# kshedden/muscato

Measured on AMD Instinct MI355X. Metric: reads/sec (100 bp, multi-map) at 1/2/4/8 MI355X; confirm-kernel HBM GB/s vs peak, higher is better.
Workload: dtype u32

## Files before the change

### muscato_amd/api.py

```python
from __future__ import annotations

import ctypes
import json
from dataclasses import dataclass, field, asdict
from typing import List, Optional, Sequence, Tuple

import numpy as np

from . import _lib


class MuscatoError(RuntimeError):
    pass


@dataclass
class Config:
    ReadFileName: str = ""
    GeneFileName: str = ""
    GeneIdFileName: str = ""
    ResultsFileName: str = ""
    Windows: List[int] = field(default_factory=list)
    WindowWidth: int = 0
    BloomSize: int = 0
# ... 210 lines not shown
        self._check(self._lib.musc_reads_sort_unique(self._h, seqs_ptr, off_ptr, nreads, 1 if on_device else 0,
                                                     ctypes.byref(po), ctypes.byref(pu), ctypes.byref(nu)),
                    "musc_reads_sort_unique")
        try:
            order = np.ctypeslib.as_array(ctypes.cast(po, ctypes.POINTER(ctypes.c_uint32)), shape=(max(nreads, 1),))[:nreads].copy()
            ustart = np.ctypeslib.as_array(ctypes.cast(pu, ctypes.POINTER(ctypes.c_uint32)), shape=(nu.value + 1,)).copy()
        finally:
            self._lib.musc_free_u32(po)
            self._lib.musc_free_u32(pu)
        self.n_reads = int(nu.value)
        return order, ustart

    def load_reads_packed(self, seqs: Sequence[bytes]) -> None:
        buf, off = concat(seqs)
        packed, mask = pack_2bit(buf, int(off[-1]))
        packed = np.concatenate([packed, np.zeros(8, np.uint8)])
        mp = mask.ctypes.data if mask is not None else None
        self._check(self._lib.musc_reads_load_packed(self._h, packed.ctypes.data, mp, off.ctypes.data, len(off) - 1),
                    "musc_reads_load_packed")
        self.n_reads = len(off) - 1

    def load_reads_packed_ptr(self, bases_ptr: int, mask_ptr: int, off_ptr: int, nreads: int) -> None:
        self._check(self._lib.musc_reads_load_packed(self._h, bases_ptr, mask_ptr or None, off_ptr, nreads),
                    "musc_reads_load_packed")
        self.n_reads = nreads

    def load_reads_packed32_ptr(self, bases_ptr: int, mask_ptr: int, lengths_ptr: int, fixed_len: int, nreads: int,
                                async_upload: bool = False) -> None:
        self._check(self._lib.musc_reads_load_packed32(self._h, bases_ptr, mask_ptr or None, lengths_ptr or None,
                                                       fixed_len, nreads, 1 if async_upload else 0),
                    "musc_reads_load_packed32")
        self.n_reads = nreads

    def match_device(self, cfg: Config, apply_mmtol: bool = True, skip_block_check: bool = False,
                     n_shards: int = 1) -> int:
        p = cfg.to_params(apply_mmtol, skip_block_check, n_shards)
        self._apply_partition_bases(cfg)
        n = ctypes.c_uint64()
        self._check(self._lib.musc_match_device(self._h, ctypes.byref(p), ctypes.byref(n)), "musc_match_device")
        return int(n.value)

    def hits_to(self, ptr: int, capacity: int, on_device: bool) -> None:
        self._check(self._lib.musc_hits_copy(self._h, ptr, capacity, 1 if on_device else 0), "musc_hits_copy")

    def hits_to_packed(self, ptr: int, capacity: int, on_device: bool, bits: Sequence[int], read_base: int = 0) -> None:
        b = (ctypes.c_int32 * 4)(*bits)
        self._check(self._lib.musc_hits_copy_packed(self._h, ptr, capacity, 1 if on_device else 0, read_base, b),
                    "musc_hits_copy_packed")

    def hits_to_compact(self, words_ptr: int, words_cap: int, counts_ptr: int, counts_cap: int, on_device: bool,
                        bits: Sequence[int]) -> None:
        b = (ctypes.c_int32 * 3)(*bits)
        self._check(self._lib.musc_hits_copy_compact(self._h, words_ptr, words_cap, counts_ptr, counts_cap,
                                                     1 if on_device else 0, b), "musc_hits_copy_compact")

    def unpack_hits(self, src_ptr: int, n: int, on_device: bool, bits: Sequence[int], dst_ptr: int) -> None:
        b = (ctypes.c_int32 * 4)(*bits)
        self._check(self._lib.musc_hits_unpack(self._h, src_ptr, n, 1 if on_device else 0, b, dst_ptr), "musc_hits_unpack")

    def match(self, cfg: Config, apply_mmtol: bool = True, n_shards: int = 1) -> np.ndarray:
        n = self.match_device(cfg, apply_mmtol, n_shards=n_shards)
        out = np.zeros((n, 4), dtype=np.uint32)
        if n:
            self.hits_to(out.ctypes.data, n, False)
        return out

    def overflow_probes(self) -> np.ndarray:
        pr, pw, n = ctypes.c_void_p(), ctypes.c_void_p(), ctypes.c_uint64()
        self._check(self._lib.musc_overflow_probes(self._h, ctypes.byref(pr), ctypes.byref(pw), ctypes.byref(n)),
                    "musc_overflow_probes")
        out = np.zeros((n.value, 2), dtype=np.uint32)
        if n.value:
            out[:, 0] = np.ctypeslib.as_array(ctypes.cast(pr, ctypes.POINTER(ctypes.c_uint32)), shape=(n.value,))
            out[:, 1] = np.ctypeslib.as_array(ctypes.cast(pw, ctypes.POINTER(ctypes.c_uint32)), shape=(n.value,))
        self._lib.musc_free_u32(pr)
        self._lib.musc_free_u32(pw)
        return out

    def last_instance(self) -> dict:
        w = (ctypes.c_uint32 * 4)()
        self._check(self._lib.musc_last_instance(self._h, w), "musc_last_instance")
        return {"path": "fused" if w[0] else "two-kernel" if w[1] else "none",
                "match": decode_instance(w[0]), "screen": decode_instance(w[1]), "confirm": decode_instance(w[2]),
                "block_mode": w[3] & 0xFF, "exact_rerun": bool(w[3] & 0x100)}

    def stats(self) -> dict:
        s = _lib.MuscStats()
        self._check(self._lib.musc_get_stats(self._h, ctypes.byref(s)), "musc_get_stats")
        return {k: getattr(s, k) for k, _ in s._fields_}


_INST_FIELDS = {1: ("k_match_t", ("W", "XM", "WIDE", "SG")), 2: ("k_match_g", (None, None, None, "SG")),
                3: ("k_screen", ("mask", "one", "lines")), 4: ("k_screen_t", ()), 5: ("k_confirm", ("mask", "w2"))}


def decode_instance(word: int) -> Optional[dict]:
    if not word:
        return None
    name, fields = _INST_FIELDS[word & 0xFF]
    d = {"kernel": name, "RW": (word >> 8) & 0xFF}
    for i, f in enumerate(fields):
        if f:
            d[f] = (word >> (16 + 4 * i)) & 0xF
    return d


def instance_name(d: Optional[dict]) -> str:
    return "none" if d is None else "%s<%s>" % (d["kernel"], ", ".join(str(v) for k, v in d.items() if k != "kernel"))


def instances() -> List[dict]:
    lib = _lib.load()
    n = ctypes.c_uint32()
    if lib.musc_instances(None, 0, ctypes.byref(n)):
        raise RuntimeError("musc_instances failed")
    buf = (ctypes.c_uint32 * max(1, n.value))()
    lib.musc_instances(buf, n.value, ctypes.byref(n))
    return [decode_instance(w) for w in buf[:n.value]]


def stream_plan(nreads: int, fixed_len: int, batch_reads: int = 16 << 20) -> dict:
    lib = _lib.load()
    n, planned = ctypes.c_uint64(), ctypes.c_uint64()
    if lib.musc_stream_plan(nreads, fixed_len, batch_reads, None, None, 0, ctypes.byref(n), ctypes.byref(planned)):
        raise ValueError("musc_stream_plan: %d reads of %d bases is not a read set the loader takes" % (nreads, fixed_len))
    ends = np.zeros(max(1, n.value), dtype=np.uint64)
    flags = np.zeros(max(1, n.value), dtype=np.uint8)
    lib.musc_stream_plan(nreads, fixed_len, batch_reads, ends.ctypes.data, flags.ctypes.data, n.value, ctypes.byref(n),
                         ctypes.byref(planned))
    ends, flags = ends[:n.value], flags[:n.value]
    return {"piece_ends": ends, "batch_ends": ends[flags != 0], "planned_batches": int(planned.value)}


def gather(engines: Sequence["Engine"], read_bases: Sequence[int], rccl: bool = False) -> np.ndarray:
    lib = engines[0]._lib
    n = len(engines)
    arr = (ctypes.c_void_p * n)(*[e._h for e in engines])
    bases = (ctypes.c_uint64 * n)(*[int(b) for b in read_bases])
    ph, cnt = ctypes.c_void_p(), ctypes.c_uint64()
    rc = lib.musc_gather_rccl(arr, n, bases, ctypes.byref(ph), ctypes.byref(cnt)) if rccl else 1
    if rccl and rc == 2:
        raise MuscatoError("musc_gather_rccl failed (%d): %s" % (rc, lib.musc_last_error(engines[0]._h).decode()))
    if rc != 0:
        rc = lib.musc_gather(arr, n, bases, ctypes.byref(ph), ctypes.byref(cnt))
    if rc != 0:
        raise MuscatoError("musc_gather failed (%d): %s" % (rc, lib.musc_last_error(engines[0]._h).decode()))
    out = np.zeros((cnt.value, 4), dtype=np.uint32)
    if cnt.value:
        ctypes.memmove(out.ctypes.data, ph, cnt.value * 16)
    lib.musc_free_hits(ph)
    return out


def sorted_hits(a: np.ndarray) -> np.ndarray:
    if len(a) == 0:
        return a.reshape(0, 4)
    idx = np.lexsort((a[:, 3], a[:, 2], a[:, 1], a[:, 0]))
    return a[idx]
```

### muscato_amd/csrc/kernels_match_lane.hpp

```cpp
#pragma once
#include "kernels_match_lane_inst.hpp"
#if defined(MUSC_LANE_DBG) && !defined(MUSC_LANE_DBG_SLOTS)
#define MUSC_LANE_DBG_SLOTS 3
#endif

template <int RW, int NW>
DEV void read_image_n(const Rec<RW>& rec, uint32_t sh, uint32_t (&img)[NW]) {
  const uint32_t bs = sh & 31u;
#define MUSC_IMG_W(Q) (((Q) >= 0 && (Q) < RW - 1) ? rec.w[((Q) >= 0 && (Q) < RW - 1) ? (Q) : 0] : 0u)
#define MUSC_IMG_CASE(WO)                                                  \
  case WO:                                                                 \
    _Pragma("unroll") for (int j = 0; j < NW; j++) {                       \
      const uint32_t hi = MUSC_IMG_W(j - WO), lo = MUSC_IMG_W(j - WO - 1); \
      img[j] = bs ? ((hi << bs) | (lo >> (32u - bs))) : hi;                \
    }                                                                      \
    break;
  switch (__builtin_amdgcn_readfirstlane((int)(sh >> 5))) {
    MUSC_IMG_CASE(0) MUSC_IMG_CASE(1) MUSC_IMG_CASE(2) MUSC_IMG_CASE(3)
    MUSC_IMG_CASE(4) MUSC_IMG_CASE(5) MUSC_IMG_CASE(6) MUSC_IMG_CASE(7)
    MUSC_IMG_CASE(8) MUSC_IMG_CASE(9) MUSC_IMG_CASE(10) MUSC_IMG_CASE(11) MUSC_IMG_CASE(12)
    default:
#pragma unroll
      for (int j = 0; j < NW; j++) img[j] = 0u;
      break;
  }
#undef MUSC_IMG_CASE
#undef MUSC_IMG_W
}


DEV void put_tuple(uint4* __restrict__ dst, uint32_t a, uint32_t b, uint32_t c, uint32_t d) { *dst = make_uint4(a, b, c, d); }

template <int RW, int W, int XM, bool WIDE, int SG>
__global__ __launch_bounds__(TILE, MATCHT_WAVES) void k_match_t(const uint32_t* __restrict__ rd, uint64_t r0, uint32_t n,
                                                                const MatchParams* __restrict__ mp,
                                                                const uint16_t* __restrict__ nmiss_tab,
                                                                const CtxBucket* __restrict__ T, const CtxEntry* __restrict__ E,
                                                                uint4* __restrict__ stage, uint64_t stage_cap,
                                                                uint4* __restrict__ spill, uint64_t spill_cap,
                                                                uint32_t* __restrict__ tbase, uint32_t* __restrict__ tcount2,
                                                                int block_mode, uint32_t block_thr,
                                                                uint32_t* __restrict__ block_table,
                                                                unsigned long long* __restrict__ counters,
                                                                const uint32_t* __restrict__ rdx) {
  static_assert(W >= 1 && W <= CTX_MAX_W, "context buckets serve at most CTX_MAX_W windows");
  constexpr bool RX = XM != 0, DBX = XM == 2;
  constexpr int NWAVE = TILE / 64;
  constexpr int NIN = WIDE ? CTXW_INLINE : CTX_INLINE;
  constexpr uint32_t WLIST = RW >= 12 && MATCHT_WLIST > 64 ? 64u : (uint32_t)MATCHT_WLIST;
  typedef XPos<WIDE> XP;
  constexpr int NW = WIDE ? CTXW_WORDS : 8;
  constexpr int NQ = WIDE ? 3 : 2;
  constexpr int NT = WIDE ? 3 : 2;
  extern __shared__ uint32_t s_dyn[];
  __shared__ uint4 s_line[NWAVE][64 * 8];
  __shared__ __attribute__((aligned(16))) uint32_t s_rec[2][NWAVE][WT * RW];
  __shared__ uint32_t s_meta[2][NWAVE][WT];
  __shared__ uint32_t s_xp[RX ? 2 : 1][RX ? NWAVE : 1][RX ? WT : 1];
  __shared__ uint32_t s_best[2][NWAVE][WT];
  __shared__ uint3 s_list[2][NWAVE][WLIST];
  __shared__ uint32_t s_cb[NWAVE][2 * WT];
  __shared__ uint32_t s_oix[NWAVE][WT];
  __shared__ uint8_t s_own[NWAVE][WT];
  __shared__ uint16_t s_nm[CONF_NM];
  constexpr bool BB_LDS = (W == 3 && XM == 0 && RW <= 8);
  __shared__ uint32_t s_bbp[BB_LDS ? NWAVE : 1][BB_LDS ? W : 1][BB_LDS ? WT : 1];

  typedef SpecGeom<SG> SGm;
  constexpr bool SPEC = SGm::on;
  static_assert(!SPEC || (SGm::nwin == W && !WIDE && XM == 0 && SGm::ww <= 15), "a specialised instance is built for its geometry's window count, 120-base buckets, no X, a direct table of one-word keys");
  constexpr int S_WW = SGm::ww, S_CL = SGm::CL, S_L = SGm::L, S_MIND = SGm::min_dinuc;
  constexpr int S_WIN[CTX_MAX_W] = {SGm::win[0], SGm::win[1], SGm::win[2], SGm::win[3]};
  if constexpr (SPEC) {
    bool same = mp->ww == S_WW && mp->CL == S_CL && mp->min_dinuc == S_MIND && mp->direct == 1 && mp->bits == 2 * S_WW && mp->W == W;
#pragma unroll
    for (int k = 0; k < W; k++) same = same && mp->win[k] == S_WIN[k] && mp->need[k] == (1u << k) - 1u;
    if (!same) {
      if (threadIdx.x == 0) atomicOr(&counters[3], 8ull);
      return;
    }
  }
  const int ww = SPEC ? S_WW : mp->ww, CL = SPEC ? S_CL : mp->CL, min_dinuc = SPEC ? S_MIND : mp->min_dinuc,
            direct = SPEC ? 1 : mp->direct, bits = SPEC ? 2 * S_WW : mp->bits;
  const uint32_t q1zero = mp->q1zero_mask;
  int win[W];
#pragma unroll
  for (int k = 0; k < W; k++) win[k] = SPEC ? S_WIN[k] : mp->win[k];
  uint32_t* const s_sketch = s_dyn + 2 * NWAVE * WT * W;
  for (uint32_t t = threadIdx.x; t < CONF_NM; t += TILE) s_nm[t] = t <= (uint32_t)mp->max_len ? nmiss_tab[t] : (uint16_t)0;
  if (block_mode) {
    for (uint32_t t = threadIdx.x; t < 2u * NWAVE * WT * W; t += TILE) s_dyn[t] = 0;
    if (block_mode == 1)
      for (uint32_t t = threadIdx.x; t < (1u << MATCH_SKETCH_BITS); t += TILE) s_sketch[t] = 0;
  }
  s_best[0][threadIdx.x >> 6][threadIdx.x & 63] = 0xFFFFFFFFu;
  s_best[1][threadIdx.x >> 6][threadIdx.x & 63] = 0xFFFFFFFFu;
  if (blockIdx.x == 0 && threadIdx.x == 0) tcount2[(n + WT - 1) / WT] = 0;
  __syncthreads();

  const uint32_t nwt = (n + WT - 1) / WT;
  const uint32_t gw = blockIdx.x * NWAVE + (threadIdx.x >> 6), nw = gridDim.x * NWAVE;
  const uint64_t region = stage_cap / nw, region0 = region * gw;
  const uint64_t sregion = spill_cap / nw / 2, sregion_w = 2 * sregion * gw;
  uint64_t used = 0;
  uint32_t maxspill = 0;
  uint32_t nvalid = 0, ncand = 0, ncmp = 0, novf = 0, nrep = 0;
  const uint32_t mmtol = (uint32_t)mp->mmtol;
  const bool apply = mp->apply_mmtol != 0;

  auto fetch = [&](uint32_t wt, Rec<RW>& rec) __attribute__((always_inline)) {
    const uint32_t i = wt * WT + (opaque(threadIdx.x) & 63);
    rec.load(rd + (r0 + (i < n ? i : 0)) * (uint64_t)RW, RW);
  };
  auto phase_a = [&](uint32_t wt, const Rec<RW>& rec, uint32_t& xw, uint32_t (&bb)[W]) __attribute__((always_inline)) -> uint32_t {
    const uint32_t lane = opaque(threadIdx.x) & 63;
    const bool active = wt * WT + lane < n;
    const int len = (int)rec.len();
    uint32_t valid = 0;
    xw = 0;
    uint32_t xwin = 0;
    if constexpr (RX) {
      if (active && rec.has_x()) xw = rdx[r0 + wt * WT + lane];
      const uint32_t xc = XPOS_CNT(xw);
      if (xc > XP::MAX) xwin = 0xFFFFFFFFu;
#pragma unroll
      for (int k = 0; k < W; k++) {
        const uint32_t q1 = (uint32_t)win[k];
#pragma unroll
        for (int q = 0; q < (int)XP::MAX; q++)
          if ((uint32_t)q < xc && XP::at(xw, q) - q1 < (uint32_t)ww) xwin |= 1u << k;
      }
    }
    if (ww <= 16 && direct) {
      const uint32_t kmask = ww == 16 ? 0xFFFFFFFFu : ((1u << (2 * ww)) - 1u);
#pragma unroll
      for (int k = 0; k < W; k++) {
        const uint32_t q1 = (uint32_t)win[k], q2 = q1 + (uint32_t)ww;
        const uint32_t key = (uint32_t)rec.ext(2 * q1) & kmask;
        bool pt = active && (uint32_t)len >= q2 && !((xwin >> k) & 1u);
#ifdef MUSC_LANE_DBG
        if (min_dinuc > 0 && !(MUSC_LANE_DBG & 16)) pt = pt && key_dinucs16(key, ww) >= min_dinuc;
#else
        if (min_dinuc > 0) pt = pt && key_dinucs16(key, ww) >= min_dinuc;
#endif
        bb[k] = pt ? __brev(key) >> (32 - 2 * ww) : WB_NONE;
        valid |= pt ? 1u << k : 0u;
      }
    } else {
#pragma unroll
      for (int k = 0; k < W; k++) {
        uint32_t b = WB_NONE;
        const uint32_t q1 = (uint32_t)win[k], q2 = q1 + (uint32_t)ww;
        if (active) {
          bool pt = (uint32_t)len >= q2 && !((xwin >> k) & 1u);
          if (pt && min_dinuc > 0)
            pt = (ww <= 16 ? rec_count_dinuc16(rec, q1, ww) : rec_count_dinuc(rec, rec, false, q1, ww)) >= min_dinuc;
          if (pt) {
            b = rec_bucket(rec, rec, false, q1, ww, bits, direct);
            valid |= 1u << k;
          }
        }
        bb[k] = b;
      }
    }
    nvalid += __popc(valid);
    return valid;
  };
  auto issue_window = [&](uint32_t bbk, uint4 (&a)[4], uint4 (&b2)[4]) __attribute__((always_inline)) {
    const uint32_t lane = opaque(threadIdx.x) & 63;
    uint32_t bq[8];
#pragma unroll
    for (int i = 0; i < 8; i++) bq[i] = (uint32_t)__builtin_amdgcn_ds_bpermute((int)((i * 8 + (lane >> 3)) * 4), (int)bbk);
#pragma unroll
    for (int i = 0; i < 8; i++) {
      const uint32_t c = ((lane & 7u) ^ (lane >> 4) ^ ((lane >> 3) & 1u)) ^ (((uint32_t)i & 1u) << 2);
#ifdef MUSC_LANE_DBG
      if (MUSC_LANE_DBG & 2) continue;
#endif
      const u32x4_v* p = reinterpret_cast<const u32x4_v*>(T + (bq[i] != WB_NONE ? bq[i] : 0u)) + c;
      const u32x4_v x = __builtin_nontemporal_load(p);
      if (i < 4) a[i] = make_uint4(x.x, x.y, x.z, x.w);
      else b2[i - 4] = make_uint4(x.x, x.y, x.z, x.w);
    }
  };

  struct WinTab {
    uint32_t lm[NW];
    uint32_t need;
    uint32_t wm[W][NW];
// ... 253 lines not shown
          constexpr int sh1c = 2 * (S_CL - S_WIN[W - 1]);
#pragma unroll
          for (int j = 0; j < NW; j++) wm0[j] = bit_range_mask(sh1c + 2 * S_WIN[0] - 32 * j, sh1c + 2 * (S_WIN[0] + S_WW) - 32 * j);
        } else {
          const uint32_t* __restrict__ row = mp->wm[W - 1][0];
#pragma unroll
          for (int j = 0; j < NW; j++) wm0[j] = row[j];
        }
        uint32_t z = 0;
        bool ok;
        const uint32_t rem = DBX ? ctx_rem(c[NW - 1], xi != 0) : c[NW - 1] >> 16;
        if (__any(have && (jx == (uint32_t)q1 || jx == 0u))) ok = have & ctx_fit(jx, rem, q1, ww, len, &z);
        else ok = have & (jx >= (uint32_t)q1) & (len - q1 <= (int)rem);
        ncmp += ok ? 1u : 0u;
        uint32_t w = NX_REJECT;
        uint32_t tm[NW];
        target_xmask(ok, xi, c[NW - 1], gene, jx, tm);
        if (ok) {
          uint32_t ia[NW], ib[NW], xm[NW];
          read_image_n<RW, NW>(rec, sha, ia);
          read_image_n<RW, NW>(rec, shb, ib);
          x_mask(xw, sh, xm);
          uint32_t d[NW], nx = 0, acc0 = 0;
#pragma unroll
          for (int j = 0; j < NW; j++) {
            d[j] = diff_word((k1 ? ib[j] : ia[j]) ^ c[j], xm[j], tm[j], lm[j]);
            nx = bcnt_add(d[j], nx);
            if constexpr (SPEC) acc0 |= d[j] & wm0[j];
            else acc0 = and_or_s(d[j], wm0[j], acc0);
          }
          uint32_t exact = REC_VALID(meta) & (z ? ~q1zero : 0xFFFFFFFFu);
          if (k1 && acc0) exact &= ~1u;
          const uint32_t kbit = k1 ? 2u : 1u;
          if (nx <= REC_BUDGET(meta) && (exact & kbit)) {
            const bool first = (exact & (kbit - 1u)) == 0;
            w = (first ? nx : (nx | NX_DUP)) | NX_ACC0 | (k1 ? 1u << 20 : 0u) | (seg << 24);
          }
        }
        report_any(p, nl, w, gene, jx - (uint32_t)q1);
        return;
      }
      uint32_t w = NX_REJECT;
      int q1 = 0;
#pragma unroll
      for (int kk = 0; kk < W; kk++) {
        const bool mine = have && ek == (uint32_t)kk;
        if (!__any(mine)) continue;
        const int q1k = win[kk];
        const uint32_t shk = 2u * (uint32_t)(CL - q1k);
        WinTab tb;
        win_tab(ul, kk, shk, (uint32_t)len, tb);
        uint32_t img[NW], xm[NW];
        read_image_n<RW, NW>(rec, shk, img);
        x_mask(xw, shk, xm);
        const uint32_t w2 = score(mine, kk, q1k, img, tb, xm, gene, jx, xi, c, len, REC_BUDGET(meta), REC_VALID(meta), seg);
        if (mine) {
          w = w2;
          q1 = q1k;
        }
      }
      report_any(p, nl, w, gene, jx - (uint32_t)q1);
    };
    auto entry_fetch = [&]() __attribute__((always_inline)) {
      const uint32_t eix = lane < o_n ? s_oix[wid][lane] : 0u;
      const uint32_t* __restrict__ pe = reinterpret_cast<const uint32_t*>(E) + ctx_entry_word<WIDE>(eix);
#pragma unroll
      for (int q = 0; q < NQ; q++) o_q[q] = *reinterpret_cast<const u32x4_u*>(pe + 4 * q);
#pragma unroll
      for (int q = 0; q < NT; q++) o_t[q] = pe[4 * NQ + q];
    };
    auto owner_tables = [&](uint32_t c0, const uint32_t (&oc)[W], const uint32_t (&ovf)[W], const uint32_t (&pre)[W]) __attribute__((always_inline)) {
#pragma unroll
      for (int kk = 0; kk < W; kk++) {
        const uint32_t e_lo = c0 > pre[kk] ? c0 - pre[kk] : 0u;
        const uint32_t e_hi = pre[kk] + oc[kk] > c0 + WT ? (c0 + WT > pre[kk] ? c0 + WT - pre[kk] : 0u) : oc[kk];
#pragma unroll 1
        for (uint32_t e = e_lo; e < e_hi; e++) {
          s_own[wid][pre[kk] + e - c0] = (uint8_t)(kk * WT + lane);
          s_oix[wid][pre[kk] + e - c0] = ovf[kk] + e;
        }
      }
      wave_lds_sync();
    };
    auto overflow_rest_prev = [&]() __attribute__((always_inline)) {
      if (total_prev <= (uint32_t)WT) return;
      const uint32_t pp = par ^ 1u;
      uint32_t pre[W], total = 0;
#pragma unroll
      for (int kk = 0; kk < W; kk++) {
        const uint32_t inc = wave_scan_incl(oc_prev[kk]);
        pre[kk] = total + inc - oc_prev[kk];
        total += (uint32_t)__builtin_amdgcn_readlane((int)inc, 63);
      }
      for (uint32_t c0 = WT; c0 < total; c0 += WT) {
        owner_tables(c0, oc_prev, ovf_prev, pre);
        const uint32_t cnt = total - c0 < (uint32_t)WT ? total - c0 : (uint32_t)WT;
        const bool mine = lane < cnt;
        const uint32_t probe = mine ? (uint32_t)s_own[wid][lane] : 0u;
        const uint32_t eix = mine ? s_oix[wid][lane] : 0u;
        const uint32_t ek = probe >> 6, seg = probe & 63u;
        const uint32_t* __restrict__ pe = reinterpret_cast<const uint32_t*>(E) + ctx_entry_word<WIDE>(eix);
        u32x4_u tq[NQ];
        uint32_t tt[NT];
#pragma unroll
        for (int q = 0; q < NQ; q++) tq[q] = *reinterpret_cast<const u32x4_u*>(pe + 4 * q);
#pragma unroll
        for (int q = 0; q < NT; q++) tt[q] = pe[4 * NQ + q];
        Rec<RW> trec;
        trec.load(rd + (r0 + (uint64_t)wt_prev * WT + seg) * (uint64_t)RW, RW);
        const uint32_t tmeta = s_meta[pp][wid][seg];
        uint32_t txw = 0;
        if constexpr (RX) txw = s_xp[pp][wid][seg];
        wave_lds_sync();
        entry_compare(pp, nlist_prev, ulen_prev, cnt, ek, seg, tmeta, txw, trec, tq, tt);
      }
    };
    auto phase_d_prev = [&]() __attribute__((always_inline)) {
#ifdef MUSC_LANE_DBG
      if (MUSC_LANE_DBG & 8) return;
#endif
      const uint32_t pp = par ^ 1u;
      uint32_t* const best_l = s_best[pp][wid];
      uint32_t* const wcnt_l = s_dyn + (pp * NWAVE + wid) * WT * W;
      const uint32_t nl = nlist_prev;
      const uint32_t nspill = nl > WLIST ? nl - WLIST : 0u;
      const bool spill_ok = nspill <= sregion;
      if (nspill > maxspill) maxspill = nspill;
      if (nspill) asm volatile("s_waitcnt vmcnt(0)" ::: "memory");
      if (block_mode) {
#pragma unroll
        for (int k = 0; k < W; k++) {
          const uint32_t cw = (BB_LDS ? 0u : wc_prev[k]) + wcnt_l[k * WT + lane];
          wcnt_l[k * WT + lane] = 0;
          if (!cw) continue;
          const uint32_t h = block_hash32((uint32_t)k, BB_LDS ? s_bbp[BB_LDS ? wid : 0][BB_LDS ? k : 0][BB_LDS ? lane : 0] : bb_prev[k]);
          if (block_mode == 1) atomicAdd(&s_sketch[h >> (32 - MATCH_SKETCH_BITS)], cw);
          else atomicAdd(&block_table[h >> (32 - BLOCK_TABLE_BITS)], cw);
        }
      }
      const uint32_t b0 = best_l[lane];
      const uint32_t bestr = best_prev < b0 ? best_prev : b0;
      const uint32_t thr_own = apply ? bestr + mmtol : 0xFFFFu;
      const bool s0 = OWNK >= 1 && kc_prev > 0 && (k0w_prev & 0xFFFFu) <= thr_own, s1 = OWNK >= 2 && kc_prev > 1 && (k1w_prev & 0xFFFFu) <= thr_own;
      const uint32_t nown = (s0 ? 1u : 0u) + (s1 ? 1u : 0u);
      uint32_t cnum = nown;
      auto item = [&](uint32_t j, uint32_t* gene, uint32_t* pos) __attribute__((always_inline)) -> uint32_t {
        if (j < WLIST) {
          const uint3 it = s_list[pp][wid][j];
          *gene = it.y;
          *pos = it.z;
          return it.x;
        }
        const uint32_t* sp = reinterpret_cast<const uint32_t*>(spill + sregion_w + pp * sregion + (j - WLIST));
        *gene = __hip_atomic_load(sp + 1, __ATOMIC_RELAXED, __HIP_MEMORY_SCOPE_AGENT);
        *pos = __hip_atomic_load(sp + 2, __ATOMIC_RELAXED, __HIP_MEMORY_SCOPE_AGENT);
        return __hip_atomic_load(sp, __ATOMIC_RELAXED, __HIP_MEMORY_SCOPE_AGENT);
      };
      const uint32_t nuse = spill_ok ? nl : (nl < WLIST ? nl : WLIST);
      uint32_t kw = NX_REJECT, kg = 0, kp = 0, ko = 0;
      if (nuse) {
        best_l[lane] = bestr;
        cnt_l[lane] = 0;
        wave_lds_sync();
        if (lane < nuse) {
          const uint32_t w = item(lane, &kg, &kp);
          const uint32_t rl = w >> 24;
          const uint32_t thr = apply ? best_l[rl] + mmtol : 0xFFFFu;
          if ((w & 0xFFFFu) <= thr) {
            kw = w;
            ko = atomicAdd(&cnt_l[rl], 1u);
          }
        }
        for (uint32_t j = 64 + lane; j < nuse; j += 64) {
          uint32_t g, p;
          const uint32_t w = item(j, &g, &p);
          const uint32_t rl = w >> 24;
          const uint32_t thr = apply ? best_l[rl] + mmtol : 0xFFFFu;
          if ((w & 0xFFFFu) <= thr) atomicAdd(&cnt_l[rl], 1u);
        }
        wave_lds_sync();
        cnum += cnt_l[lane];
      }
      const uint32_t inc = wave_scan_incl(cnum);
      const uint32_t total = __builtin_amdgcn_readlane(inc, 63);
      const uint32_t mybase = inc - cnum;
      const uint64_t base = region0 + used;
      const bool fits = spill_ok && used + total <= region;
      if (lane == 0) {
        tbase[wt_prev] = (uint32_t)base;
        tcount2[wt_prev] = fits ? total : 0u;
      }
      if (fits && total) {
        const uint32_t rid = (uint32_t)(r0 + wt_prev * WT + lane);
        if (s0) put_tuple(&stage[base + mybase], rid, k0g_prev, k0p_prev, k0w_prev & 0xFFFFu);
        if (s1) put_tuple(&stage[base + mybase + (s0 ? 1u : 0u)], rid, k1g_prev, k1p_prev, k1w_prev & 0xFFFFu);
        if (nuse) {
          base_l[lane] = mybase + nown;
          wave_lds_sync();
          if (kw != NX_REJECT) {
            const uint32_t rl = kw >> 24;
            put_tuple(&stage[base + base_l[rl] + ko], (uint32_t)(r0 + wt_prev * WT + rl), kg, kp, kw & 0xFFFFu);
          }
          if (nuse > 64) {
            for (uint32_t j = 64 + lane; j < nuse; j += 64) {
              uint32_t g, p;
              const uint32_t w = item(j, &g, &p);
              const uint32_t rl = w >> 24, v = w & 0xFFFFu;
              const uint32_t thr = apply ? best_l[rl] + mmtol : 0xFFFFu;
              if (v > thr) continue;
              const uint32_t ord = atomicAdd(&cnt_l[rl], 0xFFFFFFFFu) - 1u;
              put_tuple(&stage[base + base_l[rl] + ord], (uint32_t)(r0 + wt_prev * WT + rl), g, p, v);
            }
          }
        }
      }
      wave_lds_sync();
      best_l[lane] = 0xFFFFFFFFu;
      used += total;
      nrep += kc_prev < (uint32_t)OWNK ? kc_prev : (uint32_t)OWNK;
      nrep += lane == 0 ? nl : 0u;
    };
    auto finish_prev = [&]() __attribute__((always_inline)) {
      entry_compare(par ^ 1u, nlist_prev, ulen_prev, o_n, o_k, o_seg, o_meta, o_xw, o_rec, o_q, o_t);
      PF(6)
      overflow_rest_prev();
      wave_lds_sync();
      phase_d_prev();
      PF(7)
    };

    uint32_t nlist = 0;
    uint32_t kc = 0, k0w = NX_REJECT, k0g = 0, k0p = 0, k1w = NX_REJECT, k1g = 0, k1p = 0;
    uint32_t best = 0xFFFFFFFFu;
    uint32_t ulen = 0xFFFFFFFFu, total_cur = 0;
    uint32_t wc[W], oc[W], ovf[W];
    uint32_t meta_nx = 0, xw_nx = 0, bb_nx[W];
#pragma unroll
    for (int k = 0; k < W; k++) wc[k] = oc[k] = ovf[k] = 0, bb_nx[k] = WB_NONE;

    if (have_cur) {
      const bool active = wt * WT + lane < n;
      const int rlen = (int)REC_LEN(meta_cur);
      const uint32_t budget = REC_BUDGET(meta_cur), valid_cur = REC_VALID(meta_cur);
      s_meta[par][wid][lane] = meta_cur;
      if constexpr (RX) s_xp[par][wid][lane] = xw_cur;
      const uint32_t len0 = (uint32_t)__builtin_amdgcn_readfirstlane(rlen);
      ulen = __ballot(active && (uint32_t)rlen != len0) == 0 ? len0 : 0xFFFFFFFFu;

      uint3* const list_cur = s_list[par][wid];
      auto report_own = [&](uint32_t w, uint32_t gene, uint32_t pos, uint32_t& wck) __attribute__((always_inline)) {
        const bool acc = w != NX_REJECT;
        wck += acc ? 1u : 0u;
        const bool rep = acc && !(w & NX_DUP);
        const bool first = OWNK >= 1 && rep && kc == 0, second = OWNK >= 2 && rep && kc == 1, later = rep && kc >= (uint32_t)OWNK;
        k0w = first ? w : k0w; k0g = first ? gene : k0g; k0p = first ? pos : k0p;
        k1w = second ? w : k1w; k1g = second ? gene : k1g; k1p = second ? pos : k1p;
        kc += rep ? 1u : 0u;
        const uint32_t v = w & 0xFFFFu;
        best = rep && v < best ? v : best;
        const unsigned long long vote = __ballot(later);
        if (vote == 0) return;
        const uint32_t below = __builtin_amdgcn_mbcnt_hi((uint32_t)(vote >> 32), __builtin_amdgcn_mbcnt_lo((uint32_t)vote, 0u));
        const uint32_t slot = nlist + below;
        nlist += (uint32_t)__popcll(vote);
        if (!later) return;
        if (slot < WLIST) {
          list_cur[slot] = make_uint3(w, gene, pos);
        } else if (slot - WLIST < sregion) {
          spill[sregion_w + par * sregion + (slot - WLIST)] = make_uint4(w, gene, pos, 0u);
        }
      };

      auto window = [&](auto kc) __attribute__((always_inline)) {
        constexpr int k = decltype(kc)::value;
        const int q1 = win[k];
        const uint32_t sh = 2u * (uint32_t)(CL - q1);
        WinTab tb;
        win_tab(ulen, k, sh, (uint32_t)rlen, tb);
        {
#pragma unroll
          for (int i = 0; i < 8; i++) line_l[i * 64 + lane] = i < 4 ? va[i] : vb[i - 4];
        }
        PF(0)
        if (k == 0 && have_prev) entry_fetch();
        if (W == 1) {
          if (have_prev) finish_prev();
          if (have_next) phase_a_all(wt + nw, par ^ 1u, rec_nx, meta_nx, xw_nx, bb_nx);
          wave_lds_sync();
        }
        if (k + 1 < W) {
          issue_window(bb_cur[k + 1 < W ? k + 1 : 0], va, vb);
        } else {
          if (have_next) issue_window(bb_nx[0], va, vb);
          if (wt + 2 * nw < nwt) fetch(wt + 2 * nw, rec_nx);
// ... 74 lines not shown
            const bool live = cnt > 0u;
            if (__any(live)) {
              const uint4 c2 = line_l[rb ^ 2u], c3 = line_l[rb ^ 3u];
              const uint32_t c[NW] = {h1.x, h1.y, h1.z, h1.w, c2.x, c2.y, c2.z, c2.w, c3.x, c3.y, c3.z, c3.w, m4.x};
              const uint32_t xi = DBX && (h0.w & CTX_XFLAG) ? 0x100u | (h0.z >> 24) : 0u;
              const uint32_t gene = xi ? h0.z & 0xFFFFFFu : h0.z, jx = DBX ? h0.w & ~CTX_XFLAG : h0.w;
              const uint32_t w = score(live, k, q1, img, tb, xm, gene, jx, xi, c, rlen, budget, valid_cur, lane);
              report_own(w, gene, jx - (uint32_t)q1, wc[k]);
            }
          }
          {
            const bool live = cnt > 1u;
            if (__any(live)) {
              const uint4 c5 = line_l[rb ^ 5u], c6 = line_l[rb ^ 6u], c7 = line_l[rb ^ 7u];
              const uint32_t c[NW] = {m4.w, c5.x, c5.y, c5.z, c5.w, c6.x, c6.y, c6.z, c6.w, c7.x, c7.y, c7.z, c7.w};
              const uint32_t xi = DBX && (m4.z & CTX_XFLAG) ? 0x100u | (m4.y >> 24) : 0u;
              const uint32_t gene = xi ? m4.y & 0xFFFFFFu : m4.y, jx = DBX ? m4.z & ~CTX_XFLAG : m4.z;
              const uint32_t w = score(live, k, q1, img, tb, xm, gene, jx, xi, c, rlen, budget, valid_cur, lane);
              report_own(w, gene, jx - (uint32_t)q1, wc[k]);
            }
          }
        }
        PF(4)
      };
      window(std::integral_constant<int, 0>{});
      if constexpr (W > 1) window(std::integral_constant<int, 1>{});
      if constexpr (W > 2) window(std::integral_constant<int, 2>{});
      if constexpr (W > 3) window(std::integral_constant<int, 3>{});
#ifdef MUSC_LANE_PROF
      pf_tiles++;
#endif
    } else {
      entry_fetch();
      finish_prev();
    }
    wave_lds_sync();
    have_prev = have_cur;
    if (have_cur) {
      wt_prev = wt;
      nlist_prev = nlist;
      best_prev = best;
      kc_prev = kc; k0w_prev = k0w; k0g_prev = k0g; k0p_prev = k0p; k1w_prev = k1w; k1g_prev = k1g; k1p_prev = k1p;
      ulen_prev = ulen;
      total_prev = total_cur;
#pragma unroll
      for (int k = 0; k < W; k++) {
        if constexpr (BB_LDS) {
          const uint32_t ln = opaque(threadIdx.x) & 63;
          s_bbp[wid][k][ln] = bb_cur[k];
          if (block_mode) s_dyn[(par * NWAVE + wid) * WT * W + k * WT + ln] += wc[k];
        } else {
          bb_prev[k] = bb_cur[k];
          wc_prev[k] = wc[k];
        }
        bb_cur[k] = bb_nx[k], oc_prev[k] = oc[k], ovf_prev[k] = ovf[k];
      }
      meta_cur = meta_nx;
      xw_cur = xw_nx;
      par ^= 1u;
      wt += nw;
    }
    wave_lds_sync();
    PF(5)
  }
#ifdef MUSC_LANE_PROF
  if ((gw % 37) == 0 && (threadIdx.x & 63) == 0 && pf_tiles > 4) printf("fin %u %u %llu %llu\n", gw, pf_tiles, pstart, (unsigned long long)__builtin_amdgcn_s_memtime());
  if ((gw == 0 || gw == 1001) && (threadIdx.x & 63) == 0 && pf_tiles > 4)
    printf("wave %u: %u tiles, cycles/tile: total %llu | arrive(wait+lds write) %llu issue %llu hdr %llu phA %llu finish_prev(epass %llu rest+phD %llu) expand %llu img %llu slots %llu end %llu\n", gw, pf_tiles,
           (__builtin_amdgcn_s_memtime() - pstart) / pf_tiles, pf[0] / pf_tiles, pf[1] / pf_tiles, pf[2] / pf_tiles, pf[8] / pf_tiles,
           pf[6] / pf_tiles, pf[7] / pf_tiles, pf[3] / pf_tiles, pf[9] / pf_tiles, pf[4] / pf_tiles, pf[5] / pf_tiles);
#endif
  {
    __shared__ unsigned long long s_red[NWAVE][8];
    unsigned long long v[5] = {nvalid, ncmp, ncand, novf, nrep};
#pragma unroll
    for (int q = 0; q < 5; q++)
      for (int d = 32; d; d >>= 1) v[q] += __shfl_xor(v[q], d);
    const uint32_t wv = threadIdx.x >> 6;
    if ((threadIdx.x & 63) == 0) {
#pragma unroll
      for (int q = 0; q < 5; q++) s_red[wv][q] = v[q];
      s_red[wv][5] = used <= region ? used : 0;
      s_red[wv][6] = used;
      s_red[wv][7] = ((unsigned long long)(used > region) << 32) | maxspill;
    }
    __syncthreads();
    if (threadIdx.x == 0) {
      unsigned long long t[6] = {0, 0, 0, 0, 0, 0}, mx_used = 0, mx_spill = 0, over = 0;
      for (int w = 0; w < NWAVE; w++) {
        for (int q = 0; q < 6; q++) t[q] += s_red[w][q];
        mx_used = s_red[w][6] > mx_used ? s_red[w][6] : mx_used;
        const unsigned long long sp = s_red[w][7] & 0xFFFFFFFFull;
        mx_spill = sp > mx_spill ? sp : mx_spill;
        over |= s_red[w][7] >> 32;
      }
      if (t[0]) atomicAdd(&counters[8 + 0], t[0]);
      if (t[1]) atomicAdd(&counters[8 + 1], t[1]);
      if (t[2]) atomicAdd(&counters[8 + 3], t[2]);
      if (t[3]) atomicAdd(&counters[8 + 4], t[3]);
      if (t[4]) atomicAdd(&counters[1], t[4]);
      if (t[5]) atomicAdd(&counters[8 + 6], t[5]);
      atomicMax(&counters[8 + 7], mx_used);
      if (mx_spill) atomicMax(&counters[8 + 5], mx_spill);
      if (over) atomicOr(&counters[3], 1ull);
      if (mx_spill > sregion) atomicOr(&counters[3], 4ull);
    }
  }
  if (block_mode == 1) {
    __syncthreads();
    uint32_t hot = 0;
    for (uint32_t t = threadIdx.x; t < (1u << MATCH_SKETCH_BITS); t += TILE) hot |= s_sketch[t] >= block_thr;
    if (__any(hot) && (threadIdx.x & 63) == 0) atomicOr(&counters[6], 1ull);
  }
}
```

### muscato_amd/csrc/muscato_hip.hip

```cpp

#include <hip/hip_runtime.h>
#include <rccl/rccl.h>
#include <dlfcn.h>

#include <algorithm>
#include <cstdarg>
#include <cstdio>
#include <cstdlib>
#include <cstring>
#include <map>
#include <mutex>
#include <string>
#include <type_traits>
#include <vector>

#include "../../include/muscato_hip.h"

#include "kernels_common.hpp"
#include "kernels_index.hpp"
#include "kernels_screen.hpp"
#include "kernels_confirm.hpp"
#include "kernels_match.hpp"
#include "kernels_match_lane_inst.hpp"
#include "kernels_screen_lane.hpp"
// ... 1722 lines not shown
        HIPCHK(c, hipMemcpyAsync(&c->h_pinned[0], c->counters, 16 * 8, hipMemcpyDeviceToHost, c->stream));
        HIPCHK(c, hipStreamSynchronize(c->stream));
        const uint64_t need_stage = c->h_pinned[8 + 7] * swaves, need_spill = 2 * c->h_pinned[8 + 5] * swaves;
        if (need_stage > (1ull << 31)) {
          if (n == 1) return fail(c, 6, "one read has %llu tuples (> 2^31)", (unsigned long long)c->h_pinned[8 + 7]);
          bsz = n / 2;
          streamed = false;
          again = true;
          break;
        }
        if (c->h_pinned[3] & 8ull)
          return fail(c, 12, "internal: the kernel instance specialised for geometry %d refused this run's parameters", c->spec_geom);
        if (c->h_pinned[3] || need_stage > c->stage.cap || need_spill > c->spill.cap) {
          if (need_stage > c->stage.cap && (rc = ensure(c, c->stage, need_stage + need_stage / 4 + swaves))) return rc;
          if (need_spill > c->spill.cap && (rc = ensure(c, c->spill, need_spill + need_spill / 4 + swaves))) return rc;
          again = true;
          break;
        }
        n_windows += c->h_pinned[8 + 0];
        n_cmp += c->h_pinned[8 + 1];
        n_cand += c->h_pinned[8 + 3];
        n_ovf += c->h_pinned[8 + 4];
        if ((rc = ensure(c, c->hits, c->h_pinned[2] + c->h_pinned[8 + 6], true))) return rc;
      }
      Range rgc("scan + k_compact_w");
      tm.begin(4);
      tm.begin(1);
      rc = scan_u32(c, c->tcount2.p, c->tpre.p, (uint64_t)ntiles + 1, false, c->scan_tmp.p, c->stream);
      if (rc) return rc;
      tm.end(1);
      hipLaunchKernelGGL(k_compact_w, dim3(std::min(nblk(ntiles, 4), 4u * MAX_GRID)), dim3(256), 0, c->stream, ntiles,
                         c->bs[0].tbase.p, c->tcount2.p, c->tpre.p, c->stage.p, reinterpret_cast<uint4*>(c->hits.p),
                         c->hits.cap, c->counters);
      HIPCHK(c, hipGetLastError());
      hipLaunchKernelGGL(k_advance, dim3(1), dim3(64), 0, c->stream, c->tpre.p, ntiles, c->counters);
      HIPCHK(c, hipGetLastError());
      tm.end(4);
      r0 += n;
    }
    if (again) continue;
    c->last_pp = pp;
    c->last_max_matches = (uint32_t)max_matches;
    c->last_exact_blocks = block_mode == 2;
    if (!replay) {
      if (block_mode == 2) {
        hipLaunchKernelGGL(k_block_overflow, dim3(1024), dim3(256), 0, c->stream, c->block_table.p, (uint32_t)max_matches,
                           c->counters);
        HIPCHK(c, hipGetLastError());
      }
      if (!capture) HIPCHK(c, hipEventRecord(ev1, c->stream));
      HIPCHK(c, hipMemcpyAsync(c->h_pinned, c->counters, 16 * 8, hipMemcpyDeviceToHost, c->stream));
    }
    if (capture) {
      hipGraph_t g = nullptr;
      hipError_t ge = cap.end(&g);
      if (ge == hipSuccess) ge = hipGraphInstantiate(&c->graph_exec, g, nullptr, nullptr, 0);
      if (g) (void)hipGraphDestroy(g);
      if (ge != hipSuccess) {
        (void)hipGetLastError();
        c->graph_exec = nullptr;
        c->graph_failed = true;
        return match_index_pass(c, P, nhits);
      }
      c->graph_epoch = c->data_epoch;
      c->graph_params = *P;
      c->graph_block_mode = block_mode;
      c->graph_batches = c->stats.n_batches;
    }
    if (capture || replay) {
      c->stats.n_batches = c->stats.match_launches = c->graph_batches;
      HIPCHK(c, hipEventRecord(ev0, c->stream));
      HIPCHK(c, hipGraphLaunch(c->graph_exec, c->stream));
      HIPCHK(c, hipEventRecord(ev1, c->stream));
    }
    HIPCHK(c, hipStreamSynchronize(c->stream));
    if (c->h_pinned[3] & 8ull)
      return fail(c, 12, "internal: the kernel instance specialised for geometry %d refused this run's parameters", c->spec_geom);
    if (c->h_pinned[3]) {
      if (!sized) return fail(c, 12, "internal: a capacity guard fired although every batch was sized (flags %llu)",
                              (unsigned long long)c->h_pinned[3]);
      c->sized_epoch = 0;
      return match_index_pass(c, P, nhits);
    }
    if (sized) {
      n_windows = c->h_pinned[8 + 0];
      n_cmp = c->h_pinned[8 + 1];
      n_cand = c->h_pinned[8 + 3];
      n_ovf = c->h_pinned[8 + 4];
    }
    c->stats.n_read_windows = n_windows;
    c->stats.n_candidates = n_cand;
    c->stats.n_pairs = n_cmp;
    c->stats.n_descriptors = 0;
    c->stats.n_overflow_entries = n_ovf;
    c->stats.n_accepted = c->h_pinned[1];
    c->stats.n_hits = c->nhits = c->h_pinned[2];
    c->stats.n_overflow_blocks = check_blocks ? c->h_pinned[5] : ~0ull;
    if (block_mode == 1 && (c->h_pinned[6] || c->stats.n_batches > planned_batches)) {
      c->force_exact_blocks = true;
      c->exact_epoch = c->data_epoch;
      c->exact_params = *P;
      rc = match_index_pass(c, P, nhits);
      c->force_exact_blocks = false;
      return rc;
    }
    c->stats.ms_screen = tm.total(0);
    c->stats.ms_scan = tm.total(1);
    c->stats.ms_select = tm.total(4);
    (void)hipEventElapsedTime(&c->stats.ms_total, ev0, ev1);
    const uint64_t rec_b = (2 * L + 7) / 8;
    const uint64_t ent_b = c->idx_wide ? sizeof(CtxEntryW) : sizeof(CtxEntry);
    c->stats.match_bytes = c->nreads * rec_b + n_windows * sizeof(CtxBucket) + n_ovf * ent_b + 16 * c->stats.n_hits;
    c->stats.match_bytes_strict = c->nreads * rec_b + n_windows * 8 + n_cand * ent_b + 16 * c->stats.n_hits;
    if (nhits) *nhits = c->nhits;
    c->sized_epoch = streamed ? 0 : c->data_epoch;
    c->sized_params = *P;
    c->sized_exact_blocks = block_mode == 2;
    c->sized_bsz = bsz;
    return 0;
  }
}

int musc_match_device(musc_ctx* c, const musc_params* P, uint64_t* nhits) {
  if (!c) return 1;
  const int rc = match_device_impl(c, P, nhits);
  if (rc != 0 && c->up.active && c->up.s_up) (void)hipStreamSynchronize(c->up.s_up);
  return rc;
}

static int match_partitioned(musc_ctx* c, const musc_params* P, uint64_t* nhits);

static int match_device_impl(musc_ctx* c, const musc_params* P, uint64_t* nhits) {
  Range rg_pass("musc_match_device");
  int rc = check_params(c, P);
  if (rc) return rc;
  if (!c->db2) return fail(c, 4, "no database loaded");
  if (!c->rd && c->nreads) return fail(c, 4, "no reads loaded");
  HIPCHK(c, hipSetDevice(c->device));
  if ((rc = plan_partitions(c, P, c->max_len))) return rc;
  c->cur_part = 0;
  if (c->part_first.size() > 2) return match_partitioned(c, P, nhits);
  return match_index_pass(c, P, nhits);
}

static int match_index_pass(musc_ctx* c, const musc_params* P, uint64_t* nhits) {
  int rc = ensure_index(c, P, c->max_len);
  if (rc) return rc;

  const float keep_index_ms = c->stats.ms_index_build;
  memset(&c->stats, 0, sizeof c->stats);
  c->stats.ms_index_build = keep_index_ms;
  c->stats.n_reads = c->nreads;
  c->nhits = 0;
  if (nhits) *nhits = 0;

  PathParams pp;
  memset(&pp, 0, sizeof pp);
  pp.W = P->n_windows;
  pp.ww = P->window_width;
  pp.min_dinuc = P->min_dinuc;
  pp.bits = c->idx_bits;
  pp.direct = c->idx_direct;
  pp.mmtol = P->mmtol > 0xFFFF ? 0xFFFF : P->mmtol;
  pp.apply_mmtol = P->apply_mmtol;
  pp.wide = c->wide;
  pp.max_len = (int32_t)c->max_len;
// ... 878 lines not shown
```

Baseline: 2.094 billion.

## Add uniform-owner run path with prefetch and wave-aggregated LDS counters in match kernel

When a whole 64-entry chunk of overflow entries belongs to one read window, the match kernel now scores it through a specialised run loop. That loop hoists the read image and window tables once, and can software-pipeline the entry loads one chunk ahead. The list-counting and staging passes batch several spill items per lane and replace per-lane LDS atomics with one wave-aggregated atomic when all lanes share a read. A per-instance constexpr table chooses which of these optimisations are enabled, and a flag reports when the run path fired. The cost is higher register pressure and code size, and the per-geometry table is hand-tuned.

```diff
diff --git a/muscato_amd/api.py b/muscato_amd/api.py
--- a/muscato_amd/api.py
+++ b/muscato_amd/api.py
@@ -316,7 +316,7 @@
         self._check(self._lib.musc_last_instance(self._h, w), "musc_last_instance")
         return {"path": "fused" if w[0] else "two-kernel" if w[1] else "none",
                 "match": decode_instance(w[0]), "screen": decode_instance(w[1]), "confirm": decode_instance(w[2]),
-                "block_mode": w[3] & 0xFF, "exact_rerun": bool(w[3] & 0x100)}
+                "block_mode": w[3] & 0xFF, "exact_rerun": bool(w[3] & 0x100), "long_runs": bool(w[3] & 0x200)}
 
     def stats(self) -> dict:
         s = _lib.MuscStats()
diff --git a/muscato_amd/csrc/kernels_match_lane.hpp b/muscato_amd/csrc/kernels_match_lane.hpp
--- a/muscato_amd/csrc/kernels_match_lane.hpp
+++ b/muscato_amd/csrc/kernels_match_lane.hpp
@@ -28,6 +28,20 @@
 #undef MUSC_IMG_W
 }
 
+
+constexpr int runs_level(int RW, int W, int XM, bool WIDE, int SG) {
+  const int key = RW * 1000 + W * 100 + XM * 10 + (WIDE ? 1 : 0);
+  constexpr int off[] = {8310, 8220, 4320, 4420, 4211, 4411, 4221, 4421, 12310, 12220, 12320, 8211, 8221, 16401, 16311, 16221, 16421};
+  constexpr int l0[] = {4410, 8421, 12211, 12321, 12421};
+  constexpr int l1[] = {4401, 12401, 16211};
+  for (int k : off)
+    if (k == key) return -1;
+  for (int k : l0)
+    if (k == key) return 0;
+  for (int k : l1)
+    if (k == key) return 1;
+  return 2;
+}
 
 DEV void put_tuple(uint4* __restrict__ dst, uint32_t a, uint32_t b, uint32_t c, uint32_t d) { *dst = make_uint4(a, b, c, d); }
 
@@ -48,6 +62,12 @@
   constexpr int NWAVE = TILE / 64;
   constexpr int NIN = WIDE ? CTXW_INLINE : CTX_INLINE;
   constexpr uint32_t WLIST = RW >= 12 && MATCHT_WLIST > 64 ? 64u : (uint32_t)MATCHT_WLIST;
+#ifdef MUSC_RUNS_LEVEL
+  constexpr int RUNS_LEVEL = MUSC_RUNS_LEVEL;
+#else
+  constexpr int RUNS_LEVEL = runs_level(RW, W, XM, WIDE, SG);
+#endif
+  constexpr bool PF2 = RUNS_LEVEL >= 2;
   typedef XPos<WIDE> XP;
   constexpr int NW = WIDE ? CTXW_WORDS : 8;
   constexpr int NQ = WIDE ? 3 : 2;
@@ -105,6 +125,7 @@
   uint64_t used = 0;
   uint32_t maxspill = 0;
   uint32_t nvalid = 0, ncand = 0, ncmp = 0, novf = 0, nrep = 0;
+  uint32_t long_runs = 0;
   const uint32_t mmtol = (uint32_t)mp->mmtol;
   const bool apply = mp->apply_mmtol != 0;
 
@@ -524,6 +545,105 @@
       }
       wave_lds_sync();
     };
+    auto uniform_run = [&](auto kc, uint32_t o, uint32_t& c0, uint32_t total, uint32_t pre_o, uint32_t oc_o, uint32_t ovf_o) __attribute__((always_inline)) {
+      constexpr int kk = decltype(kc)::value;
+      const uint32_t pp = par ^ 1u;
+      const uint32_t r_end = pre_o + oc_o;
+      const uint32_t meta = (uint32_t)__builtin_amdgcn_readfirstlane((int)s_meta[pp][wid][o]);
+      uint32_t xw = 0;
+      if constexpr (RX) xw = (uint32_t)__builtin_amdgcn_readfirstlane((int)s_xp[pp][wid][o]);
+      const int len = (int)REC_LEN(meta);
+      const int q1 = win[kk];
+      const uint32_t sh = 2u * (uint32_t)(CL - q1);
+      WinTab tb;
+      win_tab(ulen_prev, kk, sh, (uint32_t)len, tb);
+      uint32_t img[NW], xm[NW];
+      {
+        Rec<RW> urec;
+        urec.load(rd + (r0 + (uint64_t)(uint32_t)__builtin_amdgcn_readfirstlane((int)wt_prev) * WT + o) * (uint64_t)RW, RW);
+        read_image_n<RW, NW>(urec, sh, img);
+      }
+      x_mask(xw, sh, xm);
+      const uint32_t* __restrict__ eb = reinterpret_cast<const uint32_t*>(E);
+      auto issue = [&](uint32_t cc, u32x4_u (&q)[NQ], uint32_t (&t)[NT]) __attribute__((always_inline)) {
+        const uint32_t cn = total - cc < (uint32_t)WT ? total - cc : (uint32_t)WT;
+        const uint32_t* __restrict__ pe = eb + ctx_entry_word<WIDE>(ovf_o + (cc - pre_o) + (lane < cn ? lane : 0u));
+#pragma unroll
+        for (int i = 0; i < NQ; i++) q[i] = *reinterpret_cast<const u32x4_u*>(pe + 4 * i);
+#pragma unroll
+        for (int i = 0; i < NT; i++) t[i] = pe[4 * NQ + i];
+      };
+      auto keep = [&](uint32_t x) __attribute__((always_inline)) -> uint32_t {
+        uint32_t y;
+        asm volatile("v_mov_b32 %0, %1" : "=v"(y) : "v"(x));
+        return y;
+      };
+      uint32_t pw = NX_REJECT, pg = 0, ppos = 0, pslot = 0;
+      auto flush = [&]() __attribute__((always_inline)) {
+        if (pw != NX_REJECT) {
+          if (pslot < WLIST) {
+            s_list[pp][wid][pslot] = make_uint3(pw, pg, ppos);
+          } else if (pslot - WLIST < sregion) {
+            spill[sregion_w + pp * sregion + (pslot - WLIST)] = make_uint4(pw, pg, ppos, 0u);
+          }
+        }
+      };
+      uint32_t nacc = 0, rbest = 0xFFFFFFFFu;
+      u32x4_u nq[NQ];
+      uint32_t nt[NT];
+      if (PF2) issue(c0, nq, nt);
+      for (;;) {
+        const uint32_t cnt = total - c0 < (uint32_t)WT ? total - c0 : (uint32_t)WT;
+        const uint32_t cn = c0 + (uint32_t)WT;
+        const uint32_t cnt_n = cn < total ? (total - cn < (uint32_t)WT ? total - cn : (uint32_t)WT) : 0u;
+        const bool more = cnt_n != 0 && cn + cnt_n <= r_end;
+        u32x4_u eq[NQ];
+        uint32_t et[NT];
+        if (PF2) {
+          asm volatile("s_waitcnt vmcnt(0)" ::: "memory");
+#pragma unroll
+          for (int i = 0; i < NQ; i++) eq[i] = u32x4_u{keep(nq[i].x), keep(nq[i].y), keep(nq[i].z), keep(nq[i].w)};
+#pragma unroll
+          for (int i = 0; i < NT; i++) et[i] = keep(nt[i]);
+          flush();
+          if (more) issue(cn, nq, nt);
+        } else {
+          issue(c0, eq, et);
+        }
+        const bool have = lane < cnt;
+        const uint32_t xi = DBX && (eq[0].y & CTX_XFLAG) ? 0x100u | (eq[0].x >> 24) : 0u;
+        const uint32_t gene = xi ? eq[0].x & 0xFFFFFFu : eq[0].x, jx = DBX ? eq[0].y & ~CTX_XFLAG : eq[0].y;
+        uint32_t c[NW];
+#pragma unroll
+        for (int j = 0; j < NW; j++) {
+          const int wi = j + 2;
+          c[j] = wi < 4 * NQ ? (wi % 4 == 0 ? eq[wi / 4].x : wi % 4 == 1 ? eq[wi / 4].y : wi % 4 == 2 ? eq[wi / 4].z : eq[wi / 4].w) : et[wi - 4 * NQ];
+        }
+        const uint32_t w = score(have, kk, q1, img, tb, xm, gene, jx, xi, c, len, REC_BUDGET(meta), REC_VALID(meta), o);
+        const bool acc = w != NX_REJECT;
+        nacc += (uint32_t)__popcll(__ballot(acc));
+        const bool rep = acc && !(w & NX_DUP);
+        const unsigned long long vote = __ballot(rep);
+        const uint32_t below = __builtin_amdgcn_mbcnt_hi((uint32_t)(vote >> 32), __builtin_amdgcn_mbcnt_lo((uint32_t)vote, 0u));
+        pslot = nlist_prev + below;
+        nlist_prev += (uint32_t)__popcll(vote);
+        pw = rep ? w : NX_REJECT;
+        pg = gene;
+        ppos = jx - (uint32_t)q1;
+        rbest = rep && (w & 0xFFFFu) < rbest ? (w & 0xFFFFu) : rbest;
+        if (!PF2) flush();
+        c0 = cn;
+        if (!more) break;
+      }
+      if (PF2) flush();
+      if (block_mode && nacc && lane == 0) atomicAdd(&s_dyn[(pp * NWAVE + wid) * WT * W + kk * WT + o], nacc);
+      for (int d = 32; d; d >>= 1) {
+        const uint32_t ob = (uint32_t)__shfl_xor((int)rbest, d);
+        rbest = ob < rbest ? ob : rbest;
+      }
+      if (lane == 0 && rbest != 0xFFFFFFFFu) atomicMin(&s_best[pp][wid][o], rbest);
+      long_runs = 1u;
+    };
     auto overflow_rest_prev = [&]() __attribute__((always_inline)) {
       if (total_prev <= (uint32_t)WT) return;
       const uint32_t pp = par ^ 1u;
@@ -534,9 +654,28 @@
         pre[kk] = total + inc - oc_prev[kk];
         total += (uint32_t)__builtin_amdgcn_readlane((int)inc, 63);
       }
-      for (uint32_t c0 = WT; c0 < total; c0 += WT) {
-        owner_tables(c0, oc_prev, ovf_prev, pre);
+      auto try_run = [&](auto kc, uint32_t& c0) __attribute__((always_inline)) -> bool {
+        constexpr int kk = decltype(kc)::value;
         const uint32_t cnt = total - c0 < (uint32_t)WT ? total - c0 : (uint32_t)WT;
+        const unsigned long long own = __ballot(pre[kk] <= c0 && pre[kk] + oc_prev[kk] >= c0 + cnt);
+        if (own == 0) return false;
+        const int o = __builtin_ctzll(own);
+        uniform_run(kc, (uint32_t)o, c0, total, (uint32_t)__builtin_amdgcn_readlane((int)pre[kk], o),
+                    (uint32_t)__builtin_amdgcn_readlane((int)oc_prev[kk], o), (uint32_t)__builtin_amdgcn_readlane((int)ovf_prev[kk], o));
+        return true;
+      };
+      for (uint32_t c0 = WT; c0 < total;) {
+        if constexpr (RUNS_LEVEL >= 0) {
+          bool ran = try_run(std::integral_constant<int, 0>{}, c0);
+          if constexpr (W > 1) ran = ran || try_run(std::integral_constant<int, 1>{}, c0);
+          if constexpr (W > 2) ran = ran || try_run(std::integral_constant<int, 2>{}, c0);
+          if constexpr (W > 3) ran = ran || try_run(std::integral_constant<int, 3>{}, c0);
+          if (ran) continue;
+        }
+        const uint32_t c_this = c0;
+        c0 += WT;
+        owner_tables(c_this, oc_prev, ovf_prev, pre);
+        const uint32_t cnt = total - c_this < (uint32_t)WT ? total - c_this : (uint32_t)WT;
         const bool mine = lane < cnt;
         const uint32_t probe = mine ? (uint32_t)s_own[wid][lane] : 0u;
         const uint32_t eix = mine ? s_oix[wid][lane] : 0u;
@@ -598,6 +737,11 @@
         *pos = __hip_atomic_load(sp + 2, __ATOMIC_RELAXED, __HIP_MEMORY_SCOPE_AGENT);
         return __hip_atomic_load(sp, __ATOMIC_RELAXED, __HIP_MEMORY_SCOPE_AGENT);
       };
+      auto item_w = [&](uint32_t j) __attribute__((always_inline)) -> uint32_t {
+        if (j < WLIST) return s_list[pp][wid][j].x;
+        return __hip_atomic_load(reinterpret_cast<const uint32_t*>(spill + sregion_w + pp * sregion + (j - WLIST)), __ATOMIC_RELAXED, __HIP_MEMORY_SCOPE_AGENT);
+      };
+      constexpr int DG = RUNS_LEVEL >= 1 ? 4 : 1;
       const uint32_t nuse = spill_ok ? nl : (nl < WLIST ? nl : WLIST);
       uint32_t kw = NX_REJECT, kg = 0, kp = 0, ko = 0;
       if (nuse) {
@@ -613,12 +757,37 @@
             ko = atomicAdd(&cnt_l[rl], 1u);
           }
         }
-        for (uint32_t j = 64 + lane; j < nuse; j += 64) {
-          uint32_t g, p;
-          const uint32_t w = item(j, &g, &p);
-          const uint32_t rl = w >> 24;
-          const uint32_t thr = apply ? best_l[rl] + mmtol : 0xFFFFu;
-          if ((w & 0xFFFFu) <= thr) atomicAdd(&cnt_l[rl], 1u);
+        if constexpr (RUNS_LEVEL < 0) {
+          for (uint32_t j = 64 + lane; j < nuse; j += 64) {
+            uint32_t g, p;
+            const uint32_t w = item(j, &g, &p);
+            const uint32_t rl = w >> 24;
+            const uint32_t thr = apply ? best_l[rl] + mmtol : 0xFFFFu;
+            if ((w & 0xFFFFu) <= thr) atomicAdd(&cnt_l[rl], 1u);
+          }
+        } else
+        for (uint32_t j0 = 64; j0 < nuse; j0 += 64 * DG) {
+          uint32_t iw[DG];
+#pragma unroll
+          for (int g = 0; g < DG; g++) {
+            const uint32_t j = j0 + 64u * g + lane;
+            iw[g] = j < nuse ? item_w(j) : NX_REJECT;
+          }
+#pragma unroll
+          for (int g = 0; g < DG; g++) {
+            if (j0 + 64u * g >= nuse) break;
+            const bool valid = j0 + 64u * g + lane < nuse;
+            const uint32_t rl = valid ? iw[g] >> 24 : 0u;
+            const uint32_t thr = apply ? best_l[rl] + mmtol : 0xFFFFu;
+            const bool pass = valid && (iw[g] & 0xFFFFu) <= thr;
+            const uint32_t rl0 = (uint32_t)__builtin_amdgcn_readfirstlane((int)rl);
+            if (__ballot(valid && rl != rl0) == 0) {
+              const uint32_t pc = (uint32_t)__popcll(__ballot(pass));
+              if (lane == 0 && pc) atomicAdd(&cnt_l[rl0], pc);
+            } else if (pass) {
+              atomicAdd(&cnt_l[rl], 1u);
+            }
+          }
         }
         wave_lds_sync();
         cnum += cnt_l[lane];
@@ -644,14 +813,46 @@
             put_tuple(&stage[base + base_l[rl] + ko], (uint32_t)(r0 + wt_prev * WT + rl), kg, kp, kw & 0xFFFFu);
           }
           if (nuse > 64) {
-            for (uint32_t j = 64 + lane; j < nuse; j += 64) {
-              uint32_t g, p;
-              const uint32_t w = item(j, &g, &p);
-              const uint32_t rl = w >> 24, v = w & 0xFFFFu;
-              const uint32_t thr = apply ? best_l[rl] + mmtol : 0xFFFFu;
-              if (v > thr) continue;
-              const uint32_t ord = atomicAdd(&cnt_l[rl], 0xFFFFFFFFu) - 1u;
-              put_tuple(&stage[base + base_l[rl] + ord], (uint32_t)(r0 + wt_prev * WT + rl), g, p, v);
+            if constexpr (RUNS_LEVEL < 0) {
+              for (uint32_t j = 64 + lane; j < nuse; j += 64) {
+                uint32_t g, p;
+                const uint32_t w = item(j, &g, &p);
+                const uint32_t rl = w >> 24, v = w & 0xFFFFu;
+                const uint32_t thr = apply ? best_l[rl] + mmtol : 0xFFFFu;
+                if (v > thr) continue;
+                const uint32_t ord = atomicAdd(&cnt_l[rl], 0xFFFFFFFFu) - 1u;
+                put_tuple(&stage[base + base_l[rl] + ord], (uint32_t)(r0 + wt_prev * WT + rl), g, p, v);
+              }
+            } else
+            for (uint32_t j0 = 64; j0 < nuse; j0 += 64 * DG) {
+              uint32_t iw[DG], ig[DG], ip[DG];
+#pragma unroll
+              for (int g = 0; g < DG; g++) {
+                const uint32_t j = j0 + 64u * g + lane;
+                ig[g] = ip[g] = 0;
+                iw[g] = j < nuse ? item(j, &ig[g], &ip[g]) : NX_REJECT;
+              }
+#pragma unroll
+              for (int g = 0; g < DG; g++) {
+                if (j0 + 64u * g >= nuse) break;
+                const bool valid = j0 + 64u * g + lane < nuse;
+                const uint32_t rl = valid ? iw[g] >> 24 : 0u, v = iw[g] & 0xFFFFu;
+                const uint32_t thr = apply ? best_l[rl] + mmtol : 0xFFFFu;
+                const bool pass = valid && v <= thr;
+                const uint32_t rl0 = (uint32_t)__builtin_amdgcn_readfirstlane((int)rl);
+                uint32_t ord = 0;
+                if (__ballot(valid && rl != rl0) == 0) {
+                  const unsigned long long vote = __ballot(pass);
+                  const uint32_t pc = (uint32_t)__popcll(vote);
+                  uint32_t old = 0;
+                  if (lane == 0 && pc) old = atomicAdd(&cnt_l[rl0], 0u - pc);
+                  old = (uint32_t)__builtin_amdgcn_readfirstlane((int)old);
+                  ord = old - 1u - __builtin_amdgcn_mbcnt_hi((uint32_t)(vote >> 32), __builtin_amdgcn_mbcnt_lo((uint32_t)vote, 0u));
+                } else if (pass) {
+                  ord = atomicAdd(&cnt_l[rl], 0xFFFFFFFFu) - 1u;
+                }
+                if (pass) put_tuple(&stage[base + base_l[rl] + ord], (uint32_t)(r0 + wt_prev * WT + rl), ig[g], ip[g], v);
+              }
             }
           }
         }
@@ -892,17 +1093,18 @@
       for (int q = 0; q < 5; q++) s_red[wv][q] = v[q];
       s_red[wv][5] = used <= region ? used : 0;
       s_red[wv][6] = used;
-      s_red[wv][7] = ((unsigned long long)(used > region) << 32) | maxspill;
+      s_red[wv][7] = ((unsigned long long)(used > region) << 32) | ((unsigned long long)(long_runs != 0) << 33) | maxspill;
     }
     __syncthreads();
     if (threadIdx.x == 0) {
-      unsigned long long t[6] = {0, 0, 0, 0, 0, 0}, mx_used = 0, mx_spill = 0, over = 0;
+      unsigned long long t[6] = {0, 0, 0, 0, 0, 0}, mx_used = 0, mx_spill = 0, over = 0, runs = 0;
       for (int w = 0; w < NWAVE; w++) {
         for (int q = 0; q < 6; q++) t[q] += s_red[w][q];
         mx_used = s_red[w][6] > mx_used ? s_red[w][6] : mx_used;
         const unsigned long long sp = s_red[w][7] & 0xFFFFFFFFull;
         mx_spill = sp > mx_spill ? sp : mx_spill;
-        over |= s_red[w][7] >> 32;
+        over |= (s_red[w][7] >> 32) & 1ull;
+        runs |= (s_red[w][7] >> 33) & 1ull;
       }
       if (t[0]) atomicAdd(&counters[8 + 0], t[0]);
       if (t[1]) atomicAdd(&counters[8 + 1], t[1]);
@@ -913,6 +1115,7 @@
       atomicMax(&counters[8 + 7], mx_used);
       if (mx_spill) atomicMax(&counters[8 + 5], mx_spill);
       if (over) atomicOr(&counters[3], 1ull);
+      if (runs) atomicOr(&counters[7], 1ull);
       if (mx_spill > sregion) atomicOr(&counters[3], 4ull);
     }
   }
diff --git a/muscato_amd/csrc/muscato_hip.hip b/muscato_amd/csrc/muscato_hip.hip
--- a/muscato_amd/csrc/muscato_hip.hip
+++ b/muscato_amd/csrc/muscato_hip.hip
@@ -1828,6 +1828,7 @@
       c->sized_epoch = 0;
       return match_index_pass(c, P, nhits);
     }
+    if (c->h_pinned[7]) c->last_inst[3] |= 0x200u;
     if (sized) {
       n_windows = c->h_pinned[8 + 0];
       n_cmp = c->h_pinned[8 + 1];
```

New measurement: 2.081 billion. About the same (-0.6%).
